# ay-lab/mustache

Measured on AMD Instinct MI355X. Metric: scale-space Mpix/s (sigma-stack+local-max), higher is better.
Workload: dtype f64

## Files before the change

### mustache_amd/csrc/mst_diff.hip

```cpp
#include <cmath>
#include <cstring>
#include <vector>
#include "mst_common.h"
#include "mst_fir.h"

namespace {

constexpr int kThreads = 256;
constexpr int kParts = 256;

__global__ void __launch_bounds__(kThreads)
diff_image_kernel(const double *__restrict__ c1, const double *__restrict__ c2, const uint8_t *__restrict__ nz1,
                  const uint8_t *__restrict__ nz2, int64_t npx, double *__restrict__ cd, uint8_t *__restrict__ nzb,
                  uint32_t *__restrict__ count) {
    const int b = blockIdx.y;
    const int64_t base = (int64_t)b * npx;
    uint32_t local = 0;
    const int64_t stride = (int64_t)gridDim.x * blockDim.x;
    for (int64_t i = (int64_t)blockIdx.x * blockDim.x + threadIdx.x; i < npx; i += stride) {
        const bool t = nz1[base + i] && nz2[base + i];
        cd[base + i] = t ? c1[base + i] - c2[base + i] : 0.0;
        nzb[base + i] = t ? 1 : 0;
        local += t ? 1u : 0u;
    }
#pragma unroll
    for (int o = 32; o > 0; o >>= 1) local += __shfl_xor(local, o, 64);
    if ((threadIdx.x & 63) == 0 && local) atomicAdd(count + b, local);
}

template <int MODE>
__global__ void __launch_bounds__(kThreads)
masked_partial_kernel(const double *__restrict__ a, const double *__restrict__ bimg, const uint8_t *__restrict__ mask,
                      int64_t npx, const double *__restrict__ fit, double *__restrict__ partial) {
    __shared__ double sh[kThreads];
    const int b = blockIdx.y;
    const int64_t base = (int64_t)b * npx;
    const double mean = MODE == 1 ? fit[2 * b] : 0.0;
    double acc = 0.0;
    const int64_t stride = (int64_t)gridDim.x * blockDim.x;
    for (int64_t i = (int64_t)blockIdx.x * blockDim.x + threadIdx.x; i < npx; i += stride) {
        if (mask[base + i]) {
            const double d = a[base + i] - bimg[base + i];
            if (MODE == 0) acc = acc + d;
            else { const double t = d - mean; acc = acc + t * t; }
        }
    }
    sh[threadIdx.x] = acc;
    __syncthreads();
    for (int s = kThreads / 2; s > 0; s >>= 1) {
        if ((int)threadIdx.x < s) sh[threadIdx.x] = sh[threadIdx.x] + sh[threadIdx.x + s];
        __syncthreads();
    }
    if (threadIdx.x == 0) partial[(size_t)b * kParts + blockIdx.x] = sh[0];
}

template <int MODE>
__global__ void __launch_bounds__(kParts)
masked_finish_kernel(const double *__restrict__ partial, const uint32_t *__restrict__ count, double *__restrict__ fit) {
    __shared__ double sh[kParts];
    const int b = blockIdx.x;
    sh[threadIdx.x] = partial[(size_t)b * kParts + threadIdx.x];
    __syncthreads();
    for (int s = kParts / 2; s > 0; s >>= 1) {
        if ((int)threadIdx.x < s) sh[threadIdx.x] = sh[threadIdx.x] + sh[threadIdx.x + s];
        __syncthreads();
    }
    if (threadIdx.x == 0) {
        const double n = (double)count[b];
        if (MODE == 0) fit[2 * b] = sh[0] / n;
        else fit[2 * b + 1] = sqrt(sh[0] / n);
    }
}

__device__ __forceinline__ double ndtr(double a) {
    const double x = a * 0.70710678118654752440;
    const double z = fabs(x);
    if (z < 0.70710678118654752440) return 0.5 + 0.5 * erf(x);
    double y = 0.5 * erfc(z);
    if (x > 0) y = 1.0 - y;
    return y;
}

__global__ void __launch_bounds__(kThreads)
pair_pvalue_kernel(const mst_found *__restrict__ found, uint32_t found_cap, const uint32_t *__restrict__ found_count,
                   const double *__restrict__ g2, const double *__restrict__ g3, const double *__restrict__ fit,
                   int B, int64_t npx, int tested_per_octave, int sample_offset, double *__restrict__ ppair) {
    const int b = blockIdx.y;
    const int fb = b + sample_offset;
    const uint32_t n = found_count[fb];
    if (n > found_cap) return;
    for (uint32_t i = blockIdx.x * blockDim.x + threadIdx.x; i < n; i += gridDim.x * blockDim.x) {
        const mst_found rec = found[(size_t)fb * found_cap + i];
        const int oct = ((int)rec.level - 1) / tested_per_octave;
        const size_t at = ((size_t)oct * B + b) * npx + rec.pixel;
        const double x = g2[at] - g3[at];
        const double loc = fit[2 * ((size_t)oct * B + b)], scale = fit[2 * ((size_t)oct * B + b) + 1];
        double cdf = ndtr((x - loc) / scale);
        if (!isfinite(cdf)) cdf = 1.0;
        if (cdf > 0.5) cdf = 1.0 - cdf;
        ppair[(size_t)fb * found_cap + i] = cdf * 2.0;
    }
}


struct DiffLevels {
    int n_octaves;
    int radius[16][2];
    double taps[16][2][MST_MAX_RADIUS + 1];
};

template <class T, int R>
__device__ __forceinline__ void diff_blur(const double *ct, double *vb, const double (&w)[T::RMAX + 1], int tid,
                                          const double *vsrc, double *vdst, const double *hsrc, double (&g)[T::K]) {
    vpass<T, R>(ct, vb, w, tid, vsrc, vdst, 0);
    __syncthreads();
    hpass<T, R>(hsrc, w, g);
    __syncthreads();
}

template <class T>
__device__ __forceinline__ void diff_blur_dispatch(int r, const double *ct, double *vb, const double (&w)[T::RMAX + 1],
                                                   int tid, const double *vsrc, double *vdst, const double *hsrc,
                                                   double (&g)[T::K]) {
#define MST_CASE(R_)                                                                  \
    case R_:                                                                          \
        if constexpr (R_ <= T::RMAX) diff_blur<T, R_>(ct, vb, w, tid, vsrc, vdst, hsrc, g); \
        break;
    switch (r) {
        MST_CASE(1) MST_CASE(2) MST_CASE(3) MST_CASE(4) MST_CASE(5) MST_CASE(6) MST_CASE(7)
        MST_CASE(8) MST_CASE(9) MST_CASE(10) MST_CASE(11) MST_CASE(12) MST_CASE(13) MST_CASE(14)
        MST_CASE(15) MST_CASE(16) MST_CASE(17) MST_CASE(18) MST_CASE(19) MST_CASE(20) MST_CASE(21)
        MST_CASE(22) MST_CASE(23) MST_CASE(24) MST_CASE(25) MST_CASE(26) MST_CASE(27) MST_CASE(28)
        default: break;
    }
#undef MST_CASE
}


struct BandSource {
    const double *band1, *band2;
    int64_t n;
    int dpx;
    const int64_t *starts;
    const int32_t *tile_list;

    __device__ __forceinline__ int tile_of(int slot) const { return tile_list[slot]; }

    template <class T>
    __device__ __forceinline__ void stage(int b, int Y0, int X0, int CH, double *ct, uint8_t *nzb, int tid) const {
        constexpr int RGR = T::RGR, RGC = T::RGC, RMAX = T::RMAX;
        const int64_t start = starts[b];
        const int dpx = this->dpx;
        const int64_t n = this->n;
        const bool inner = Y0 >= 0 && X0 >= 0 && Y0 + T::CTR <= CH && X0 + T::CTC <= CH;
        auto pixel = [&](double r1, double r2, int off, double &val, bool &both) {
            const bool fill = off <= 4 || off >= dpx + 1;
            both = r1 != 0.0 && r2 != 0.0 && off >= 4;
            val = both ? ((fill ? 2.0 : r1) - (fill ? 2.0 : r2)) : 0.0;
        };
        if (inner) {
            constexpr int ND = T::CTR + T::CTC - 1;
            constexpr int PER = (T::CTR + 63) / 64;
            constexpr int U = 10 / PER > 0 ? 10 / PER : 1;
            for (int q0 = tid >> 6; q0 < ND; q0 += T::NW * U) {
                double a1[U][PER], a2[U][PER];
#pragma unroll
                for (int u = 0; u < U; ++u) {
                    const int q = q0 + u * T::NW;
                    const int dd = q - (T::CTR - 1);
                    const int off = X0 - Y0 + dd;
                    const int i_lo = dd < 0 ? -dd : 0;
                    const int i_hi = T::CTC - dd < T::CTR ? T::CTC - dd : T::CTR;
                    const bool in_band = q < ND && off >= 0 && off <= dpx + 1;
                    const int64_t at = (int64_t)(in_band ? off : 0) * n + start + Y0;
#pragma unroll
                    for (int e = 0; e < PER; ++e) {
                        const int i = i_lo + (tid & 63) + 64 * e;
                        const bool ok = in_band && i < i_hi && start + X0 + i + dd < n;
                        a1[u][e] = ok ? band1[at + i] : 0.0;
                        a2[u][e] = ok ? band2[at + i] : 0.0;
                    }
                }
#pragma unroll
                for (int u = 0; u < U; ++u) {
                    const int q = q0 + u * T::NW;
                    if (q >= ND) break;
                    const int dd = q - (T::CTR - 1);
                    const int off = X0 - Y0 + dd;
                    const int i_lo = dd < 0 ? -dd : 0;
                    const int i_hi = T::CTC - dd < T::CTR ? T::CTC - dd : T::CTR;
#pragma unroll
                    for (int e = 0; e < PER; ++e) {
                        const int i = i_lo + (tid & 63) + 64 * e;
                        if (i >= i_hi) continue;
                        const int j = i + dd;
                        double val;
                        bool both;
                        pixel(a1[u][e], a2[u][e], off, val, both);
                        ct[j * T::CTP + i] = val;
                        const int ri = i - RMAX, rj = j - RMAX;
                        if (ri >= 0 && ri < RGR && rj >= 0 && rj < RGC) nzb[ri * RGC + rj] = both ? 1 : 0;
                    }
                }
            }
        } else {
            for (int idx = tid; idx < T::CTR * T::CTC; idx += T::NT) {
                const int i = idx / T::CTC, j = idx - i * T::CTC;
                const int uy = Y0 + i, ux = X0 + j;
                const int by = reflect_idx(uy, CH), bx = reflect_idx(ux, CH);
                const int off = bx - by;
                double r1 = 0.0, r2 = 0.0;
                if (off >= 0 && off <= dpx + 1 && start + bx < n) {
                    r1 = band1[(int64_t)off * n + start + by];
                    r2 = band2[(int64_t)off * n + start + by];
                }
                double val;
                bool both;
                pixel(r1, r2, off, val, both);
                ct[j * T::CTP + i] = val;
                const int ri = i - RMAX, rj = j - RMAX;
                if (ri >= 0 && ri < RGR && rj >= 0 && rj < RGC) {
                    const bool inside = uy >= 0 && uy < CH && ux >= 0 && ux < CH;
                    nzb[ri * RGC + rj] = (inside && both) ? 1 : 0;
                }
            }
        }
    }
};

struct DenseSource {
    const double *c1, *c2;

    __device__ __forceinline__ int tile_of(int slot) const { return slot; }

    template <class T>
    __device__ __forceinline__ void stage(int b, int Y0, int X0, int CH, double *ct, uint8_t *nzb, int tid) const {
        constexpr int RGR = T::RGR, RGC = T::RGC, RMAX = T::RMAX;
        constexpr int N = T::CTR * T::CTC;
        constexpr int U = 4;
        const double *p1 = c1 + (int64_t)b * CH * CH, *p2 = c2 + (int64_t)b * CH * CH;
        const bool inner = Y0 >= 0 && X0 >= 0 && Y0 + T::CTR <= CH && X0 + T::CTC <= CH;
        for (int i0 = tid; i0 < N; i0 += T::NT * U) {
            double a1[U], a2[U];
#pragma unroll
            for (int u = 0; u < U; ++u) {
                const int idx = i0 + u * T::NT;
                const int i = idx / T::CTC, j = idx - i * T::CTC;
                const int by = inner ? Y0 + i : reflect_idx(Y0 + i, CH), bx = inner ? X0 + j : reflect_idx(X0 + j, CH);
                const int64_t at = (int64_t)by * CH + bx;
                a1[u] = idx < N ? p1[at] : 0.0;
                a2[u] = idx < N ? p2[at] : 0.0;
            }
#pragma unroll
            for (int u = 0; u < U; ++u) {
                const int idx = i0 + u * T::NT;
                if (idx >= N) break;
                const int i = idx / T::CTC, j = idx - i * T::CTC;
                const bool both = a1[u] != 0.0 && a2[u] != 0.0;
                ct[j * T::CTP + i] = both ? a1[u] - a2[u] : 0.0;
                const int ri = i - RMAX, rj = j - RMAX;
                if (ri >= 0 && ri < RGR && rj >= 0 && rj < RGC) {
                    const int uy = Y0 + i, ux = X0 + j;
                    nzb[ri * RGC + rj] = (uy < CH && ux < CH && both) ? 1 : 0;
                }
            }
        }
    }
};

template <class T, class Src>
__global__ void __launch_bounds__(T::NT)
diff_dog_kernel(const Src src, int CH, int B, const DiffLevels *__restrict__ lv, double *__restrict__ dog,
                double *__restrict__ partial, uint32_t *__restrict__ mask_count, int tiles_x, int n_slots) {
    constexpr int K = T::K, RGR = T::RGR, RGC = T::RGC, RMAX = T::RMAX;
    extern __shared__ __align__(16) double lds[];
    double *ct = lds;
    double *vb = ct + T::CT_ELEMS;
    double *red = vb + T::VB_ELEMS;
    const int tid = threadIdx.x, b = blockIdx.y;
    const int per_xcd = gridDim.x >> 3;
    const int slot = (blockIdx.x & 7) * per_xcd + (blockIdx.x >> 3);
    if (slot >= n_slots) return;
    const int tile = src.tile_of(slot);
    const int ty = tile / tiles_x, tx = tile - ty * tiles_x;
    const int y0 = ty * RGR, x0 = tx * RGC;
    const int rr = tid % RGR, cg = tid / RGR;
    const int gy = y0 + rr;

    uint8_t *nzb = reinterpret_cast<uint8_t *>(vb);
    src.template stage<T>(b, y0 - RMAX, x0 - RMAX, CH, ct, nzb, tid);
    __syncthreads();
    uint32_t in_mask = 0, both_mask = 0;
#pragma unroll
    for (int k = 0; k < K; ++k) {
        const int gx = x0 + cg * K + k;
        if (gy < CH && gx < CH) {
            in_mask |= 1u << k;
            if (nzb[rr * RGC + cg * K + k]) both_mask |= 1u << k;
        }
    }
    uint32_t mine = __builtin_popcount(both_mask);
#pragma unroll
    for (int o = 32; o > 0; o >>= 1) mine += __shfl_xor(mine, o, 64);
    if ((tid & 63) == 0 && mine) atomicAdd(mask_count + b, mine);
    __syncthreads();

    constexpr int V_MAINC = T::NT / (T::RGR / K);
    const int v_rgp = tid / V_MAINC, v_col = tid - v_rgp * V_MAINC;
    const double *vsrc = ct + v_col * T::CTP + v_rgp * K;
    double *vdst = vb + (v_rgp * K) * T::VP + v_col;
    const double *hsrc = vb + rr * T::VP + cg * K;
    double *part = partial + (((size_t)b * n_slots + slot) * lv->n_octaves) * 2;
    for (int o = 0; o < lv->n_octaves; ++o) {
        double g2[K], g3[K];
        {
            double taps[RMAX + 1];
#pragma unroll
            for (int j = 0; j <= RMAX; ++j) taps[j] = lv->taps[o][0][j];
            diff_blur_dispatch<T>(lv->radius[o][0], ct, vb, taps, tid, vsrc, vdst, hsrc, g2);
        }
        {
            const DiffLevels *lv3 = lv;
            if constexpr (RMAX > 8) asm volatile("" : "+s"(lv3));
            double taps[RMAX + 1];
#pragma unroll
            for (int j = 0; j <= RMAX; ++j) taps[j] = lv3->taps[o][1][j];
            diff_blur_dispatch<T>(lv3->radius[o][1], ct, vb, taps, tid, vsrc, vdst, hsrc, g3);
        }
        double s1 = 0.0, s2 = 0.0;
        double *out = dog + (((size_t)o * B + b) * CH + gy) * CH + x0 + cg * K;
#pragma unroll
        for (int k = 0; k < K; ++k) {
            const double dk = g2[k] - g3[k];
            if ((in_mask >> k) & 1u) out[k] = dk;
            if ((both_mask >> k) & 1u) {
                s1 = s1 + dk;
                s2 = s2 + dk * dk;
            }
        }
        red[tid] = s1;
        red[T::NT + tid] = s2;
        __syncthreads();
        for (int st = T::NT / 2; st > 0; st >>= 1) {
            if (tid < st) {
                red[tid] = red[tid] + red[tid + st];
                red[T::NT + tid] = red[T::NT + tid] + red[T::NT + tid + st];
            }
            __syncthreads();
        }
        if (tid == 0) {
            part[2 * o] = red[0];
            part[2 * o + 1] = red[T::NT];
        }
        __syncthreads();
    }
}

__global__ void __launch_bounds__(256)
diff_fit_kernel(const double *__restrict__ partial, int ntiles, int n_slots, const int32_t *__restrict__ slot_of_tile,
                int n_oct, int B, const uint32_t *__restrict__ mask_count, double *__restrict__ fit) {
    __shared__ double sa[256], sb[256];
    const int o = blockIdx.x, b = blockIdx.y, tid = threadIdx.x;
    double a = 0.0, q = 0.0;
    for (int i = tid; i < ntiles; i += 256) {
        const int sl = slot_of_tile ? slot_of_tile[i] : i;
        if (sl < 0) continue;
        a = a + partial[(((size_t)b * n_slots + sl) * n_oct + o) * 2];
        q = q + partial[(((size_t)b * n_slots + sl) * n_oct + o) * 2 + 1];
    }
    sa[tid] = a;
    sb[tid] = q;
    __syncthreads();
    for (int st = 128; st > 0; st >>= 1) {
        if (tid < st) {
            sa[tid] = sa[tid] + sa[tid + st];
            sb[tid] = sb[tid] + sb[tid + st];
        }
        __syncthreads();
    }
    if (tid == 0) {
        const double cnt = (double)mask_count[b];
        const double loc = sa[0] / cnt;
        double var = sb[0] / cnt - loc * loc;
        if (var < 0.0) var = 0.0;
        fit[2 * ((size_t)o * B + b)] = loc;
        fit[2 * ((size_t)o * B + b) + 1] = sqrt(var);
    }
}

__global__ void __launch_bounds__(kThreads)
pair_pvalue_dog_kernel(const mst_found *__restrict__ found, uint32_t found_cap, const uint32_t *__restrict__ found_count,
                       const double *__restrict__ dog, const double *__restrict__ fit, int B, int64_t npx,
                       int tested_per_octave, int sample_offset, double *__restrict__ ppair) {
    const int b = blockIdx.y;
    const int fb = b + sample_offset;
    const uint32_t nrec = found_count[fb];
    if (nrec > found_cap) return;
    for (uint32_t i = blockIdx.x * blockDim.x + threadIdx.x; i < nrec; i += gridDim.x * blockDim.x) {
        const mst_found rec = found[(size_t)fb * found_cap + i];
        const int oct = ((int)rec.level - 1) / tested_per_octave;
        const double x = dog[((size_t)oct * B + b) * npx + rec.pixel];
        const double loc = fit[2 * ((size_t)oct * B + b)], scale = fit[2 * ((size_t)oct * B + b) + 1];
        double cdf = ndtr((x - loc) / scale);
        if (!isfinite(cdf)) cdf = 1.0;
        if (cdf > 0.5) cdf = 1.0 - cdf;
        ppair[(size_t)fb * found_cap + i] = cdf * 2.0;
    }
}

using DiffTile8 = Tile<32, 64, 8>;
using DiffTile14 = Tile<32, 64, 14>;
using DiffTile28 = Tile<32, 64, 28, 4, 1, false, true>;

static_assert(DiffTile8::RGR == DiffTile14::RGR && DiffTile14::RGR == DiffTile28::RGR && DiffTile8::RGC == DiffTile14::RGC &&
                  DiffTile14::RGC == DiffTile28::RGC,
              "the three difference tiles share one region shape");

template <class T>
size_t diff_lds_bytes() { return sizeof(double) * (size_t)(T::CT_ELEMS + T::VB_ELEMS + 2 * T::NT); }
template <class T>
int diff_tiles(int CH) { return ((CH + T::RGR - 1) / T::RGR) * ((CH + T::RGC - 1) / T::RGC); }

size_t diff_align(size_t v) { return (v + 255) / 256 * 256; }

int diff_levels(const char *who, const mst_levels *lv, DiffLevels *out, int *max_radius) {
    if (!lv || lv->n_octaves < 1 || lv->n_octaves > 16 || lv->levels_per_octave < 3 ||
        lv->n_octaves * lv->levels_per_octave > MST_MAX_LEVELS)
        return mst::fail(MST_E_ARG, "%s: bad level table (1..16 octaves, >= 3 levels each)", who);
    memset(out, 0, sizeof(*out));
    out->n_octaves = lv->n_octaves;
    int mr = 0;
    for (int o = 0; o < lv->n_octaves; ++o)
        for (int q = 0; q < 2; ++q) {
            const int l = o * lv->levels_per_octave + 1 + q;
            const int r = lv->radius[l];
            if (r < 1 || r > 28) return mst::fail(MST_E_ARG, "%s: blur radius %d outside [1, 28]", who, r);
            out->radius[o][q] = r;
            for (int j = 0; j <= r; ++j) out->taps[o][q][j] = lv->taps[l][j];
            mr = r > mr ? r : mr;
        }
    *max_radius = mr;
    return MST_OK;
}

template <class T>
int diff_tile_list(int CH, int dpx, int32_t *list) {
    const int tx = (CH + T::RGC - 1) / T::RGC, nt = diff_tiles<T>(CH);
    for (int i = 0; i < 2 * nt; ++i) list[i] = -1;
    int m = 0;
    for (int t = 0; t < nt; ++t) {
        const int y0 = (t / tx) * T::RGR, x0 = (t % tx) * T::RGC;
        const int r_hi = y0 + T::RGR - 1 < CH - 1 ? y0 + T::RGR - 1 : CH - 1;
        const int c_hi = x0 + T::RGC - 1 < CH - 1 ? x0 + T::RGC - 1 : CH - 1;
        if (c_hi - y0 >= 4 && x0 - r_hi <= dpx + 1) {
            list[(size_t)nt + t] = m;
            list[(size_t)m++] = t;
        }
    }
    return m;
}

template <class T, class Src>
int diff_dog_launch(const Src &src, const int32_t *slot_of_tile, int CH, int B, const DiffLevels *d_lv, int n_oct, double *dog,
                    double *partial, int m, uint32_t *mask_count, double *fit, hipStream_t s) {
    static unsigned long long lds_allowed = 0;
    MST_HIP(mst::allow_dynamic_lds(reinterpret_cast<const void *>(&diff_dog_kernel<T, Src>), (int)diff_lds_bytes<T>(),
                                   &lds_allowed));
    const int tx = (CH + T::RGC - 1) / T::RGC, nt = diff_tiles<T>(CH);
    if (m > 0) {
        diff_dog_kernel<T, Src><<<dim3((m + 7) / 8 * 8, B), T::NT, diff_lds_bytes<T>(), s>>>(src, CH, B, d_lv, dog, partial,
                                                                                           mask_count, tx, m);
        MST_LAUNCH_CHECK();
    }
    diff_fit_kernel<<<dim3(n_oct, B), 256, 0, s>>>(partial, nt, m, slot_of_tile, n_oct, B, mask_count, fit);
    MST_LAUNCH_CHECK();
    return MST_OK;
}

int diff_which(int max_radius) { return max_radius <= DiffTile8::RMAX ? 0 : (max_radius <= DiffTile14::RMAX ? 1 : 2); }

// ... 235 lines not shown
```

### mustache_amd/csrc/mst_fir.h

```cpp
#pragma once
#include <cstdint>
#include "mst_common.h"

#if defined(MST_PROFILE) && defined(MST_ABLATE_CT)
#define MST_VARIANT(bit_) ((MST_ABLATE_CT) & (bit_))
#elif defined(MST_PROFILE)
#define MST_VARIANT(bit_) (variant & (bit_))
#else
#define MST_VARIANT(bit_) 0
#endif

#ifdef MST_PROFILE
#define MST_TRACE_WGS 64
#define MST_TRACE_STAMPS 8
#define MST_STAMP(tr_, slot_)                                                        \
    if (tr_) {                                                                       \
        const unsigned long long t_ = __builtin_amdgcn_s_memtime();                  \
        if ((threadIdx.x & 63) == 0) (tr_)[slot_] = t_;                              \
    }
#else
#define MST_STAMP(tr_, slot_)
#endif

#ifndef MST_KC8_BELOW
// ... 27 lines not shown
#define MST_INJECT_PASS
#endif

struct DevLevels {
    int n_octaves;
    int levels_per_octave;
    int radius[MST_MAX_LEVELS];
    int first_level[16];
    double taps[MST_MAX_LEVELS][MST_MAX_RADIUS + 1];
};

constexpr int pitch_for(int need) {
    int p = need;
    while (p % 32 != 2 && p % 32 != 30) ++p;
    return p;
}
constexpr int pitch_min(int need) {
    int p = need + (need & 1);
    while ((p / 2) % 2 == 0) p += 2;
    return p;
}

template <int RGR_, int RGC_, int RMAX_, int K_ = 8, int MINW_ = 1, bool FMA_ = false, bool TIGHT_ = false>
struct Tile {
    static constexpr bool FMA = FMA_;
    static constexpr int RGR = RGR_, RGC = RGC_;
    static constexpr int ITR = RGR_ - 2, ITC = RGC_ - 2;
    static constexpr int RMAX = RMAX_;
    static constexpr int K = K_;
    static constexpr int MINW = MINW_;
    static constexpr int NCG = RGC / K;
    static constexpr int NT = RGR * NCG;
    static constexpr int NW = NT / 64;
    static constexpr int CTR = RGR + 2 * RMAX;
    static constexpr int CTC = RGC + 2 * RMAX;
    static constexpr int CTP = TIGHT_ ? pitch_min(CTR) : pitch_for(CTR);
    static constexpr int VP = TIGHT_ ? pitch_min(RGC + 2 * RMAX) : pitch_for(RGC + 2 * RMAX);
    static constexpr int CT_ELEMS = CTC * CTP;
    static constexpr int VB_ELEMS = RGR * VP;
    static constexpr int DE_ELEMS = NCG * 2 * RGR;
    static constexpr int ST_ELEMS = MST_MAX_TESTED * NW * 2;
    static constexpr size_t LDS_BYTES = sizeof(double) * (size_t)(CT_ELEMS + VB_ELEMS + DE_ELEMS + ST_ELEMS);
    static_assert(NT % 64 == 0 && RGR % K == 0 && RGC % K == 0, "whole waves, whole groups");
    static_assert(64 % RGR == 0 || RGR % 64 == 0, "a wave holds whole runs of consecutive rows");
    static_assert(CTP % 2 == 0 && VP % 2 == 0 && CT_ELEMS % 2 == 0 && VB_ELEMS % 2 == 0, "16-byte alignment");
};

__device__ __forceinline__ int reflect_idx(int i, int n) {
    const int p = 2 * n;
    i %= p;
    if (i < 0) i += p;
    return i < n ? i : p - 1 - i;
}

template <int K, int R>
__device__ __forceinline__ void fir_sym(const double (&win)[K + 2 * R], const double (&w)[R + 1], double (&t)[K]) {
#pragma unroll
    for (int k = 0; k < K; ++k) t[k] = win[k + R] * w[0];
#pragma unroll
    for (int j = R; j >= 1; --j) {
        double s[K];
#pragma unroll
        for (int k = 0; k < K; ++k) s[k] = win[k + R - j] + win[k + R + j];
#pragma unroll
        for (int k = 0; k < K; ++k) s[k] = s[k] * w[j];
#pragma unroll
        for (int k = 0; k < K; ++k) t[k] = t[k] + s[k];
    }
}

template <int K, int R>
struct Chunk {
    static constexpr int KC = (K >= 8 && R < MST_KC8_BELOW) ? 8 : (K >= 4 ? 4 : K);
};

#if defined(MST_INJECT)
#define MST_FIR_INJ_TPARAM , int INJ = 0
#define MST_FIR_INJ_PARAM , Inject *inj = nullptr
#else
#define MST_FIR_INJ_TPARAM
#define MST_FIR_INJ_PARAM
#endif
template <int KC, int R, int OFF, bool FMA MST_FIR_INJ_TPARAM>
__device__ __forceinline__ void fir_chunk(const double *__restrict__ p, const double (&w)[R + 1], double (&t)[KC] MST_FIR_INJ_PARAM) {
    constexpr int NP = (KC + 2 * R + OFF + 1) / 2;
    constexpr int QC0 = (R + OFF) >> 1, QC1 = (R + KC - 1 + OFF) >> 1;
    const double2 *p2 = reinterpret_cast<const double2 *>(p);
    double x[2 * NP];
#if defined(MST_PROFILE) && defined(MST_ABL_NOLDS)
#define MST_LD(q_)                                        \
    {                                                     \
        double a_ = w[0], b_ = w[R];                      \
        asm volatile("" : "+v"(a_), "+v"(b_));            \
        x[2 * (q_)] = a_;                                 \
        x[2 * (q_) + 1] = b_;                             \
    }
#else
#define MST_LD(q_)                     \
    {                                  \
        const double2 v_ = p2[q_];     \
        x[2 * (q_)] = v_.x;            \
        x[2 * (q_) + 1] = v_.y;        \
    }
#endif
#pragma unroll
    for (int q = QC0; q <= QC1; ++q) MST_LD(q)
#if defined(MST_INJECT)
    if constexpr (INJ == 3) {
        __builtin_amdgcn_sched_barrier(0);
        inject_work<>(*inj);
        __builtin_amdgcn_sched_barrier(0);
    }
#endif
    int lq_hi = -1, rq_lo = NP;
#pragma unroll
    for (int k = 0; k < KC; ++k) t[k] = x[R + k + OFF] * w[0];
#pragma unroll
    for (int j = R; j >= 1; --j) {
        const int lq1 = (R - j + KC - 1 + OFF) >> 1, rq0 = (R + j + OFF) >> 1;
#pragma unroll
        for (int q = 0; q < NP; ++q) {
            if (q > lq_hi && q <= lq1 && q < QC0) MST_LD(q)
            if (q < rq_lo && q >= rq0 && q > QC1) MST_LD(q)
        }
        lq_hi = lq1 > lq_hi ? lq1 : lq_hi;
        rq_lo = rq0 < rq_lo ? rq0 : rq_lo;
#if defined(MST_INJECT)
        if constexpr (INJ == 4) {
            __builtin_amdgcn_sched_barrier(0);
            inject_work<(MST_INJ_DP + R - 1) / R, (MST_INJ_INT + R - 1) / R>(*inj);
            __builtin_amdgcn_sched_barrier(0);
        }
#endif
#if defined(MST_PROFILE) && defined(MST_ABL_NOMATH)
        if (j & 1) t[j % KC] = t[j % KC] + (x[R - j + OFF] + x[R + KC - 1 + j + OFF]);
#else
        double s[KC];
#pragma unroll
        for (int k = 0; k < KC; ++k) s[k] = x[R + k - j + OFF] + x[R + k + j + OFF];
        if constexpr (FMA) {
#pragma unroll
            for (int k = 0; k < KC; ++k) t[k] = __builtin_fma(s[k], w[j], t[k]);
        } else {
#pragma unroll
            for (int k = 0; k < KC; ++k) s[k] = s[k] * w[j];
#pragma unroll
            for (int k = 0; k < KC; ++k) t[k] = t[k] + s[k];
        }
#endif
    }
#undef MST_LD
}

template <class T, int R>
__device__ __forceinline__ void vpass(const double *__restrict__ ct, double *__restrict__ vb,
                                      const double (&wall)[T::RMAX + 1], int ptid, const double *__restrict__ vsrc,
                                      double *__restrict__ vdst, int variant MST_INJECT_ARG) {
    constexpr int K = T::K, KC = Chunk<T::K, R>::KC;
    constexpr int NC = T::RGC + 2 * R;
    constexpr int NRG = T::RGR / K;
    constexpr int MAINC = T::NT / NRG < NC ? T::NT / NRG : NC;
    constexpr int OFF = (T::RMAX - R) & 1;
    double w[R + 1];
#pragma unroll
    for (int j = 0; j <= R; ++j) w[j] = wall[j];
    static_assert(MAINC == T::NT / NRG, "the main-item mapping below is radius independent");
    if (!MST_VARIANT(16)) {
        const double *p = vsrc + (T::RMAX - R) * T::CTP + (T::RMAX - R - OFF);
        double *q = vdst;
#pragma unroll
        for (int h = 0; h < K / KC; ++h) {
            double t[KC];
#if defined(MST_INJECT) && (MST_INJECT == 3 || MST_INJECT == 4)
            if (h == 0) fir_chunk<KC, R, OFF, T::FMA, MST_INJECT>(p + h * KC, w, t, &inj);
            else
#endif
            fir_chunk<KC, R, OFF, T::FMA>(p + h * KC, w, t);
#pragma unroll
            for (int k = 0; k < KC; ++k) q[(h * KC + k) * T::VP] = t[k];
        }
#if defined(MST_INJECT) && MST_INJECT == 1
        inject_work<>(inj);
#endif
    }
    if constexpr (MAINC < NC) if (!MST_VARIANT(8)) {
        constexpr int PR = 4;
        constexpr int XC = NC - MAINC;
        constexpr int XRG = T::RGR / PR;
        for (int it = ptid; it < XRG * XC; it += T::NT) {
            const int rgp = it / XC;
            const int col = MAINC + (it - rgp * XC);
            const int row0 = rgp * PR;
            const double *p = ct + ((T::RMAX - R) + col) * T::CTP + (row0 + T::RMAX - R - OFF);
            double t[PR];
            fir_chunk<PR, R, OFF, T::FMA>(p, w, t);
            double *q = vb + row0 * T::VP + col;
#pragma unroll
            for (int k = 0; k < PR; ++k) q[k * T::VP] = t[k];
        }
    }
}

template <class T, int R>
__device__ __forceinline__ void hpass(const double *__restrict__ p, const double (&wall)[T::RMAX + 1],
                                      double (&g)[T::K]) {
    constexpr int K = T::K, KC = Chunk<T::K, R>::KC;
    double w[R + 1];
#pragma unroll
    for (int j = 0; j <= R; ++j) w[j] = wall[j];
#pragma unroll
    for (int h = 0; h < K / KC; ++h) {
        double t[KC];
        fir_chunk<KC, R, 0, T::FMA>(p + h * KC, w, t);
#pragma unroll
        for (int k = 0; k < KC; ++k) g[h * KC + k] = t[k];
    }
}

}
```

### mustache_amd/csrc/mst_scale_space.hip

```cpp
#include <algorithm>
#include <climits>
#include <cmath>
#include <cstdlib>
#include <cstring>
#include <vector>
#include "mst_common.h"

#include "mst_fir.h"

namespace {

__device__ __forceinline__ double dmax(double a, double b) { return __builtin_fmax(a, b); }

__device__ __forceinline__ double lane_prev(double x) {
    const int lo = __builtin_amdgcn_update_dpp(0, __double2loint(x), 0x138, 0xf, 0xf, true);
    const int hi = __builtin_amdgcn_update_dpp(0, __double2hiint(x), 0x138, 0xf, 0xf, true);
    return __hiloint2double(hi, lo);
}
__device__ __forceinline__ double lane_next(double x) {
    const int lo = __builtin_amdgcn_update_dpp(0, __double2loint(x), 0x130, 0xf, 0xf, true);
    const int hi = __builtin_amdgcn_update_dpp(0, __double2hiint(x), 0x130, 0xf, 0xf, true);
    return __hiloint2double(hi, lo);
}

template <int CTRL, int ROW_MASK>
__device__ __forceinline__ double dpp_fetch(double x) {
    const int lo = __builtin_amdgcn_mov_dpp(__double2loint(x), CTRL, ROW_MASK, 0xf, true);
    const int hi = __builtin_amdgcn_mov_dpp(__double2hiint(x), CTRL, ROW_MASK, 0xf, true);
    return __hiloint2double(hi, lo);
}
__device__ __forceinline__ void wave_reduce_min_sum(double &mn, double &sm) {
#define MST_STEP(CTRL, MASK)                                           \
    {                                                                  \
        const double a_ = dpp_fetch<CTRL, MASK>(mn);                   \
        const double b_ = dpp_fetch<CTRL, MASK>(sm);                   \
        mn = a_ < mn ? a_ : mn;                                        \
        sm = sm + b_;                                                  \
    }
    MST_STEP(0x111, 0xf)
    MST_STEP(0x112, 0xf)
    MST_STEP(0x114, 0xf)
    MST_STEP(0x118, 0xf)
    MST_STEP(0x142, 0xa)
    MST_STEP(0x143, 0xc)
#undef MST_STEP
}

template <class T, int R>
__device__ __forceinline__ void blur_level(const double *ct, double *vb, const double (&w)[T::RMAX + 1], int tid,
                                           const double *vsrc, double *vdst, const double *hsrc, double (&g)[T::K],
                                           int variant, unsigned long long *tr MST_INJECT_ARG) {
    vpass<T, R>(ct, vb, w, tid, vsrc, vdst, variant MST_INJECT_PASS);
    MST_STAMP(tr, 1)
    __syncthreads();
    MST_STAMP(tr, 2)
    if (MST_VARIANT(32)) {
#pragma unroll
        for (int k = 0; k < T::K; ++k) g[k] = 0.0;
        return;
    }
    hpass<T, R>(hsrc, w, g);
    MST_STAMP(tr, 3)
}

template <class T>
__device__ __forceinline__ void blur_dispatch(int r, const double *ct, double *vb, const double (&wg)[T::RMAX + 1],
                                              int tid, const double *vsrc, double *vdst, const double *hsrc,
                                              double (&g)[T::K], int variant, unsigned long long *tr MST_INJECT_ARG) {
#define MST_CASE(R_)                                                  \
    case R_:                                                          \
        if constexpr (R_ <= T::RMAX) blur_level<T, R_>(ct, vb, wg, tid, vsrc, vdst, hsrc, g, variant, tr MST_INJECT_PASS); \
        break;
    switch (r) {
        MST_CASE(1) MST_CASE(2) MST_CASE(3) MST_CASE(4) MST_CASE(5) MST_CASE(6) MST_CASE(7)
        MST_CASE(8) MST_CASE(9) MST_CASE(10) MST_CASE(11) MST_CASE(12) MST_CASE(13) MST_CASE(14)
        MST_CASE(15) MST_CASE(16) MST_CASE(17) MST_CASE(18) MST_CASE(19) MST_CASE(20) MST_CASE(21)
        MST_CASE(22) MST_CASE(23) MST_CASE(24) MST_CASE(25) MST_CASE(26) MST_CASE(27) MST_CASE(28)
        default: break;
    }
#undef MST_CASE
}

struct BandSrc {
    const double *band;
    int64_t n;
    int dpx;
    const int64_t *starts;
    uint32_t *nz_count;
    const double *band2;
    int split;
};

struct WorkItem {
    int32_t y0, x0, b, delta2;
};

struct KernArgs {
    const double *c;
    const uint8_t *nz;
    BandSrc src;
    int CH;
    const DevLevels *lv;
    mst_found *found;
    uint32_t found_cap;
    uint32_t *found_count;
    double *partial;
    const WorkItem *items;
    int n_items, n_tested, skip_empty, variant;
    unsigned long long *trace;
};

template <class T, bool BAND>
__global__ void __launch_bounds__(T::NT, T::MINW)
scale_space_kernel(const double *__restrict__ c, const uint8_t *__restrict__ nz, BandSrc src, int CH,
                   const DevLevels *__restrict__ lv, mst_found *__restrict__ found, uint32_t found_cap,
                   uint32_t *__restrict__ found_count, double *__restrict__ partial, const WorkItem *__restrict__ items,
                   int n_items, int n_tested, int skip_empty, int variant, unsigned long long *__restrict__ trace) {
    constexpr int K = T::K, RGR = T::RGR, RGC = T::RGC, RMAX = T::RMAX;
    extern __shared__ __align__(16) double lds[];
    double *ct = lds;
    double *vb = ct + T::CT_ELEMS;
    double *de = vb + T::VB_ELEMS;
    double *st = de + T::DE_ELEMS;

    const int tid = threadIdx.x;
    const int per_xcd = gridDim.x >> 3;
    const int slot = (blockIdx.x & 7) * per_xcd + (blockIdx.x >> 3);
    if (slot >= n_items) return;
    const WorkItem item = items[slot];
    const int b = item.b, b2 = item.delta2 != 0 ? item.b + 1 : -1;
    const int y0 = item.y0, x0 = item.x0;

    const int rr = tid % RGR;
    const int cg = tid / RGR;
    const int gy = y0 + rr;
    const bool row_in = gy >= 0 && gy < CH;
    const bool row_own = row_in && rr >= 1 && rr <= T::ITR;
    double *part = partial + (size_t)slot * n_tested * 2;

    uint32_t in_mask = 0, nz_mask = 0;
#pragma unroll
    for (int k = 0; k < K; ++k) {
        const int gx = x0 + cg * K + k;
        if (row_in && gx >= 0 && gx < CH) in_mask |= 1u << k;
    }

    if constexpr (!BAND) {
        const double *cb = c + (size_t)b * CH * CH;
        const uint8_t *nb = nz + (size_t)b * CH * CH;
#pragma unroll
        for (int k = 0; k < K; ++k) {
            const int rc = cg * K + k;
            const int gx = x0 + rc;
            if (row_own && gx >= 0 && gx < CH && rc >= 1 && rc <= T::ITC && nb[(size_t)gy * CH + gx]) nz_mask |= 1u << k;
        }
        const int any_nz = __syncthreads_or(nz_mask != 0);
        if (!any_nz && skip_empty) {
            for (int t = tid; t < n_tested; t += T::NT) {
                part[2 * t] = INFINITY;
                part[2 * t + 1] = 0.0;
            }
            return;
        }
        constexpr int CPL = (T::CTC + 63) / 64;
        int sx[CPL];
#pragma unroll
        for (int q = 0; q < CPL; ++q) sx[q] = reflect_idx(x0 - RMAX + (tid & 63) + 64 * q, CH);
        for (int i = tid >> 6; i < T::CTR; i += T::NW) {
            const double *srow = cb + (size_t)reflect_idx(y0 - RMAX + i, CH) * CH;
#pragma unroll
            for (int q = 0; q < CPL; ++q) {
                const int j = (tid & 63) + 64 * q;
                if (j < T::CTC) ct[j * T::CTP + i] = srow[sx[q]];
            }
        }
        __syncthreads();
    } else {
        const int64_t start = src.starts[b];
        const int64_t n = src.n;
        const int dpx = src.dpx;
        const double *const bandp = b >= src.split ? src.band2 : src.band;
        uint8_t *nzb = reinterpret_cast<uint8_t *>(vb);
        const int Y0 = y0 - RMAX, X0 = x0 - RMAX;
        const bool inner = Y0 >= 0 && X0 >= 0 && Y0 + T::CTR <= CH && X0 + T::CTC <= CH;
        const bool constant = inner && (X0 + T::CTC - 1 - Y0 <= 3 || X0 - (Y0 + T::CTR - 1) >= dpx + 2);
        if (constant) {
            double2 *ct2 = reinterpret_cast<double2 *>(ct);
            for (int i = tid; i < T::CT_ELEMS / 2; i += T::NT) ct2[i] = make_double2(2.0, 2.0);
            uint4 *nz4 = reinterpret_cast<uint4 *>(nzb);
            static_assert((RGR * RGC) % 16 == 0, "nzb is cleared in 16-byte pieces");
            for (int i = tid; i < RGR * RGC / 16; i += T::NT) nz4[i] = make_uint4(0, 0, 0, 0);
        } else if (inner) {
            constexpr int ND = T::CTR + T::CTC - 1;
            constexpr int PER = (T::CTR + 63) / 64;
            constexpr int U2 = (ND + 2 * T::NW - 1) / (2 * T::NW);
            constexpr int U = U2 * PER <= 20 ? U2 : 20 / PER;
            for (int q0 = tid >> 6; q0 < ND; q0 += T::NW * U) {
                double rawv[U][PER];
#pragma unroll
                for (int u = 0; u < U; ++u) {
                    const int q = q0 + u * T::NW;
                    const int dd = q - (T::CTR - 1);
                    const int off = X0 - Y0 + dd;
                    const int i_lo = dd < 0 ? -dd : 0;
                    const int i_hi = T::CTC - dd < T::CTR ? T::CTC - dd : T::CTR;
                    const bool in_band = q < ND && off >= 0 && off <= dpx + 1;
                    const double *brow = bandp + (int64_t)(in_band ? off : 0) * n + start + Y0;
#pragma unroll
                    for (int e = 0; e < PER; ++e) {
                        const int i = i_lo + (tid & 63) + 64 * e;
                        rawv[u][e] = (in_band && i < i_hi && start + X0 + i + dd < n) ? brow[i] : 0.0;
                    }
                }
#pragma unroll
                for (int u = 0; u < U; ++u) {
                    const int q = q0 + u * T::NW;
                    if (q >= ND) break;
                    const int dd = q - (T::CTR - 1);
                    const int off = X0 - Y0 + dd;
                    const int i_lo = dd < 0 ? -dd : 0;
                    const int i_hi = T::CTC - dd < T::CTR ? T::CTC - dd : T::CTR;
                    const bool filled = off <= 4 || off >= dpx + 1;
#pragma unroll
                    for (int e = 0; e < PER; ++e) {
                        const int i = i_lo + (tid & 63) + 64 * e;
                        if (i >= i_hi) continue;
                        const int j = i + dd;
                        const double raw = rawv[u][e];
                        ct[j * T::CTP + i] = filled ? 2.0 : raw;
                        const int ri = i - RMAX, rj = j - RMAX;
                        if (ri >= 0 && ri < RGR && rj >= 0 && rj < RGC)
                            nzb[ri * RGC + rj] = (raw != 0.0 && off >= 4) ? 1 : 0;
                    }
                }
            }
        } else {
            for (int idx = tid; idx < T::CTR * T::CTC; idx += T::NT) {
                const int i = idx / T::CTC, j = idx - i * T::CTC;
                const int uy = Y0 + i, ux = X0 + j;
                const int by = reflect_idx(uy, CH), bx = reflect_idx(ux, CH);
                const int off = bx - by;
                double raw = 0.0;
                if (off >= 0 && off <= dpx + 1 && start + bx < n) raw = bandp[(int64_t)off * n + start + by];
                ct[j * T::CTP + i] = (off <= 4 || off >= dpx + 1) ? 2.0 : raw;
                const int ri = i - RMAX, rj = j - RMAX;
                if (ri >= 0 && ri < RGR && rj >= 0 && rj < RGC) {
                    const bool inside = uy >= 0 && uy < CH && ux >= 0 && ux < CH;
                    nzb[ri * RGC + rj] = (inside && raw != 0.0 && off >= 4) ? 1 : 0;
                }
            }
        }
        __syncthreads();
        uint32_t mine = 0;
#pragma unroll
        for (int k = 0; k < K; ++k) {
            const int rc = cg * K + k;
            if (row_own && ((in_mask >> k) & 1u) && rc >= 1 && rc <= T::ITC && nzb[rr * RGC + rc]) nz_mask |= 1u << k;
        }
        mine = __builtin_popcount(nz_mask);
#pragma unroll
        for (int o = 32; o > 0; o >>= 1) mine += __shfl_xor(mine, o, 64);
        if ((tid & 63) == 0 && mine) {
            atomicAdd(src.nz_count + b, mine);
            if (b2 >= 0) atomicAdd(src.nz_count + b2, mine);
        }
        const int any_nz = __syncthreads_or(nz_mask != 0);
        if (!any_nz && skip_empty) {
            for (int t = tid; t < n_tested; t += T::NT) {
                part[2 * t] = INFINITY;
                part[2 * t + 1] = 0.0;
            }
            return;
        }
    }

    double gprev[K], Dc[K], Mc[K], best[K];
    uint32_t lvl[K];
    uint32_t ep = 0, ec = 0, gp = 0;
#pragma unroll
    for (int k = 0; k < K; ++k) {
        gprev[k] = Dc[k] = Mc[k] = best[k] = 0.0;
        lvl[k] = 0;
    }
    const int wave = tid >> 6, lane = tid & 63;
    const bool wave_has_nz = __any(nz_mask != 0);
    const bool wave_all_in = __all(in_mask == (1u << K) - 1u);
    double *de_mine = de + (cg * 2) * RGR + rr;
    const double *de_left = de + ((cg > 0 ? cg - 1 : 0) * 2 + 1) * RGR + rr;
    const double *de_right = de + ((cg < T::NCG - 1 ? cg + 1 : cg) * 2) * RGR + rr;

    constexpr int V_MAINC = T::NT / (T::RGR / K);
    const int v_rgp = tid / V_MAINC, v_col = tid - v_rgp * V_MAINC;
    const double *vsrc = ct + v_col * T::CTP + v_rgp * K;
    double *vdst = vb + (v_rgp * K) * T::VP + v_col;
    const double *hsrc = vb + rr * T::VP + cg * K;

    const int n_oct = MST_VARIANT(4) ? 0 : lv->n_octaves, lpo = lv->levels_per_octave;
    const int prot = (int)(blockIdx.x >> 3) * 2 + (int)(blockIdx.x >> 11);
    int tested = 0;
#if defined(MST_INJECT)
    Inject inj;
#pragma unroll
    for (int k = 0; k < 8; ++k) {
        inj.q[k] = (double)(tid + k);
        inj.u[k] = (uint32_t)(tid * 7 + k);
    }
#endif
    unsigned long long *tr = nullptr;
#ifdef MST_PROFILE
    if (trace && slot >= 3 * (per_xcd >> 3) && slot < 3 * (per_xcd >> 3) + MST_TRACE_WGS) {
        tr = trace + ((size_t)(slot - 3 * (per_xcd >> 3)) * T::NW + (tid >> 6)) * (MST_MAX_LEVELS + 1) * MST_TRACE_STAMPS;
        MST_STAMP(tr, MST_MAX_LEVELS * MST_TRACE_STAMPS + 1)
        if ((tid & 63) == 0) tr[MST_MAX_LEVELS * MST_TRACE_STAMPS + 2] = (unsigned long long)slot | ((unsigned long long)(nz_mask != 0) << 40);
    }
#endif
    for (int o = 0; o < n_oct; ++o) {
        for (int kl = lv->first_level[o]; kl <= lpo; ++kl) {
            const int l = o * lpo + kl - 1;
            const int r = lv->radius[l];
            MST_STAMP(tr, 0)
            double taps[RMAX + 1];
#pragma unroll
            for (int j = 0; j <= RMAX; ++j) taps[j] = lv->taps[l][j];
            double g[K];
            const int ptid = (tid + 64 * ((l + prot) & 3)) & (T::NT - 1);
            blur_dispatch<T>(r, ct, vb, taps, ptid, vsrc, vdst, hsrc, g, variant, tr MST_INJECT_PASS);
            double d[K];
            if (kl >= 2) {
#pragma unroll
                for (int k = 0; k < K; ++k) d[k] = gprev[k] - g[k];
                if (!wave_all_in) {
#pragma unroll
                    for (int k = 0; k < K; ++k)
                        if (!((in_mask >> k) & 1u)) d[k] = 0.0;
                }
                de_mine[0] = d[0];
                de_mine[RGR] = d[K - 1];
            }
#pragma unroll
            for (int k = 0; k < K; ++k) gprev[k] = g[k];
            MST_STAMP(tr, 4)
            __syncthreads();
            MST_STAMP(tr, 5)
#ifdef MST_PROFILE
            unsigned long long *tr_lvl = tr;
            if (tr) tr += MST_TRACE_STAMPS;
#endif
#if defined(MST_INJECT) && MST_INJECT == 2
            inject_work<>(inj);
#endif
            if (kl < 2) continue;
            if (MST_VARIANT(1) || MST_VARIANT(32)) continue;

            uint32_t en = 0, gn = 0;
            double m[K];
            if (wave_has_nz) {
                const double dl = de_left[0], dr = de_right[0];
                double hm[K];
#pragma unroll
                for (int j = 0; j < K / 2; ++j) {
                    const double pj = dmax(d[2 * j], d[2 * j + 1]);
                    hm[2 * j] = dmax(j == 0 ? dl : d[2 * j - 1], pj);
                    hm[2 * j + 1] = dmax(pj, 2 * j + 2 == K ? dr : d[2 * j + 2]);
                }
#pragma unroll
                for (int k = 0; k < K; ++k) m[k] = dmax(dmax(lane_prev(hm[k]), hm[k]), lane_next(hm[k]));
#pragma unroll
                for (int k = 0; k < K; ++k) {
                    if (d[k] == m[k]) en |= 1u << k;
                    if (d[k] > Mc[k]) gn |= 1u << k;
                }
            } else {
#pragma unroll
                for (int k = 0; k < K; ++k) m[k] = 0.0;
            }
            if (kl >= 4) {
                double lmin = INFINITY, lsum = 0.0;
                const uint32_t code = (uint32_t)tested + 1u;
                if (wave_has_nz) {
                    const uint32_t flags = nz_mask & ec & (ep | en) & gp;
#pragma unroll
                    for (int k = 0; k < K; ++k) {
                        const bool bit = (flags & (1u << k)) != 0;
                        const bool upd = bool(int(Dc[k] > dmax(best[k], m[k])) & int(bit));
                        best[k] = upd ? Dc[k] : best[k];
                        lvl[k] = upd ? code : lvl[k];
                        const bool tz = (nz_mask & (1u << k)) != 0;
                        const double a = fabs(Dc[k]);
                        lmin = __builtin_fmin(lmin, tz ? a : INFINITY);
                        lsum = lsum + (tz ? a : 0.0);
                    }
                }
                if (wave_has_nz && !MST_VARIANT(2)) wave_reduce_min_sum(lmin, lsum);
                if (lane == 63) {
                    st[(tested * T::NW + wave) * 2] = lmin;
                    st[(tested * T::NW + wave) * 2 + 1] = lsum;
                }
                ++tested;
            }
            ep = ec;
            ec = en;
            gp = gn;
#pragma unroll
            for (int k = 0; k < K; ++k) {
                Mc[k] = m[k];
                Dc[k] = d[k];
            }
#ifdef MST_PROFILE
            MST_STAMP(tr_lvl, 6)
#endif
        }
    }

    int e_b = b, e_b2 = b2, e_x0 = x0, e_delta2 = item.delta2, e_CH = CH;
    if constexpr (T::RMAX > 14) {
        typedef const KernArgs __attribute__((address_space(4))) *KernArgsPtr;
        KernArgsPtr ka = (KernArgsPtr)__builtin_amdgcn_kernarg_segment_ptr();
        found = ka->found;
        found_cap = ka->found_cap;
        found_count = ka->found_count;
        n_tested = ka->n_tested;
        part = ka->partial + (size_t)slot * n_tested * 2;
        const WorkItem again = ka->items[slot];
        e_b = again.b;
        e_b2 = again.delta2 != 0 ? again.b + 1 : -1;
        e_x0 = again.x0;
        e_delta2 = again.delta2;
        e_CH = ka->CH;
    }
#if defined(MST_INJECT)
    {
        double qs = 0.0;
        uint32_t us = 0;
#pragma unroll
        for (int k = 0; k < 8; ++k) {
            qs += inj.q[k];
            us ^= inj.u[k];
        }
        if (qs == -1.0 && us == 0x12345u) part[0] = qs;
    }
#endif
    uint32_t my_total = 0;
    uint32_t before[K];
    uint32_t kbase[K];
#pragma unroll
    for (int k = 0; k < K; ++k) {
        const unsigned long long bal = __ballot(lvl[k] != 0);
        before[k] = __builtin_popcountll(bal & ((1ull << lane) - 1ull));
        kbase[k] = my_total;
        my_total += (uint32_t)__builtin_popcountll(bal);
    }
    uint32_t *cnt_lds = reinterpret_cast<uint32_t *>(de);
    __syncthreads();
    if (lane == 0) cnt_lds[wave] = my_total;
    __syncthreads();
    if (tid == 0) {
        uint32_t tot = 0;
        for (int w = 0; w < T::NW; ++w) {
            const uint32_t n = cnt_lds[w];
            cnt_lds[w] = tot;
            tot += n;
        }
        cnt_lds[T::NW] = tot ? atomicAdd(found_count + e_b, tot) : 0u;
        cnt_lds[T::NW + 1] = (tot && e_b2 >= 0) ? atomicAdd(found_count + e_b2, tot) : 0u;
    }
    __syncthreads();
    const uint32_t wave_base = cnt_lds[T::NW] + cnt_lds[wave];
    const uint32_t wave_base2 = cnt_lds[T::NW + 1] + cnt_lds[wave];
#pragma unroll
    for (int k = 0; k < K; ++k) {
        if (lvl[k]) {
            const uint32_t off = kbase[k] + before[k];
            mst_found rec;
            rec.pixel = (uint32_t)gy * (uint32_t)e_CH + (uint32_t)(e_x0 + cg * K + k);
            rec.level = lvl[k];
            rec.value = best[k];
            if (wave_base + off < found_cap) found[(size_t)e_b * found_cap + wave_base + off] = rec;
            if (e_b2 >= 0 && wave_base2 + off < found_cap) {
                rec.pixel = (uint32_t)(gy + e_delta2) * (uint32_t)e_CH + (uint32_t)(e_x0 + cg * K + k + e_delta2);
// ... 644 lines not shown
```

Baseline: 18030.

## Remap vertical-pass edge pieces to bank-conflict-free lane layout with precomputed addresses

Replaces the strided loop over extra (halo) column pieces in the vertical FIR pass with a fixed lane-to-piece mapping. At most one piece goes to each lane, chosen per wave, and a constexpr check proves the LDS loads and stores are free of bank conflicts. Per-thread source and destination addresses are precomputed once in a VAddr struct, and the rotating piece owner becomes a wave-uniform scalar via readfirstlane. The aim is to remove LDS bank conflicts and the loop and division overhead in the halo work, at the cost of a more rigid mapping that only holds for 8-row-group tile shapes.

```diff
diff --git a/mustache_amd/csrc/mst_diff.hip b/mustache_amd/csrc/mst_diff.hip
--- a/mustache_amd/csrc/mst_diff.hip
+++ b/mustache_amd/csrc/mst_diff.hip
@@ -110,21 +110,20 @@
 };
 
 template <class T, int R>
-__device__ __forceinline__ void diff_blur(const double *ct, double *vb, const double (&w)[T::RMAX + 1], int tid,
-                                          const double *vsrc, double *vdst, const double *hsrc, double (&g)[T::K]) {
-    vpass<T, R>(ct, vb, w, tid, vsrc, vdst, 0);
+__device__ __forceinline__ void diff_blur(const double *ct, const double (&w)[T::RMAX + 1], int pwave, const VAddr &va,
+                                          const double *hsrc, double (&g)[T::K]) {
+    vpass<T, R>(ct, w, pwave, va, 0);
     __syncthreads();
     hpass<T, R>(hsrc, w, g);
     __syncthreads();
 }
 
 template <class T>
-__device__ __forceinline__ void diff_blur_dispatch(int r, const double *ct, double *vb, const double (&w)[T::RMAX + 1],
-                                                   int tid, const double *vsrc, double *vdst, const double *hsrc,
-                                                   double (&g)[T::K]) {
+__device__ __forceinline__ void diff_blur_dispatch(int r, const double *ct, const double (&w)[T::RMAX + 1], int pwave,
+                                                   const VAddr &va, const double *hsrc, double (&g)[T::K]) {
 #define MST_CASE(R_)                                                                  \
     case R_:                                                                          \
-        if constexpr (R_ <= T::RMAX) diff_blur<T, R_>(ct, vb, w, tid, vsrc, vdst, hsrc, g); \
+        if constexpr (R_ <= T::RMAX) diff_blur<T, R_>(ct, w, pwave, va, hsrc, g); \
         break;
     switch (r) {
         MST_CASE(1) MST_CASE(2) MST_CASE(3) MST_CASE(4) MST_CASE(5) MST_CASE(6) MST_CASE(7)
@@ -305,10 +304,8 @@
     if ((tid & 63) == 0 && mine) atomicAdd(mask_count + b, mine);
     __syncthreads();
 
-    constexpr int V_MAINC = T::NT / (T::RGR / K);
-    const int v_rgp = tid / V_MAINC, v_col = tid - v_rgp * V_MAINC;
-    const double *vsrc = ct + v_col * T::CTP + v_rgp * K;
-    double *vdst = vb + (v_rgp * K) * T::VP + v_col;
+    const VAddr va = vpass_addr<T>(ct, vb, tid);
+    const int pwave = __builtin_amdgcn_readfirstlane(tid >> 6);
     const double *hsrc = vb + rr * T::VP + cg * K;
     double *part = partial + (((size_t)b * n_slots + slot) * lv->n_octaves) * 2;
     for (int o = 0; o < lv->n_octaves; ++o) {
@@ -317,7 +314,7 @@
             double taps[RMAX + 1];
 #pragma unroll
             for (int j = 0; j <= RMAX; ++j) taps[j] = lv->taps[o][0][j];
-            diff_blur_dispatch<T>(lv->radius[o][0], ct, vb, taps, tid, vsrc, vdst, hsrc, g2);
+            diff_blur_dispatch<T>(lv->radius[o][0], ct, taps, pwave, va, hsrc, g2);
         }
         {
             const DiffLevels *lv3 = lv;
@@ -325,7 +322,7 @@
             double taps[RMAX + 1];
 #pragma unroll
             for (int j = 0; j <= RMAX; ++j) taps[j] = lv3->taps[o][1][j];
-            diff_blur_dispatch<T>(lv3->radius[o][1], ct, vb, taps, tid, vsrc, vdst, hsrc, g3);
+            diff_blur_dispatch<T>(lv3->radius[o][1], ct, taps, pwave, va, hsrc, g3);
         }
         double s1 = 0.0, s2 = 0.0;
         double *out = dog + (((size_t)o * B + b) * CH + gy) * CH + x0 + cg * K;
diff --git a/mustache_amd/csrc/mst_fir.h b/mustache_amd/csrc/mst_fir.h
--- a/mustache_amd/csrc/mst_fir.h
+++ b/mustache_amd/csrc/mst_fir.h
@@ -203,10 +203,51 @@
 #undef MST_LD
 }
 
+constexpr int piece_col(int lane) { return lane & 7; }
+constexpr int piece_rgp(int lane) {
+    return 2 * (lane >> 5) + 4 * ((lane >> 4) & 1) + (((((lane & 31) + 4) >> 3) ^ (lane >> 4)) & 1);
+}
+constexpr int b128_group(int lane) {
+    const int m = lane & 31;
+    return 2 * (lane >> 5) + ((m >= 4 && m < 12) || (m >= 16 && m < 20) || m >= 28 ? 1 : 0);
+}
+constexpr bool vpass_map_ok(int ctp, int vp) {
+    unsigned long long seen = 0;
+    for (int l = 0; l < 64; ++l) {
+        const int id = piece_rgp(l) * 8 + piece_col(l);
+        if (piece_rgp(l) < 0 || piece_rgp(l) > 7 || ((seen >> id) & 1)) return false;
+        seen |= 1ull << id;
+    }
+    for (int a = 0; a < 64; ++a)
+        for (int b = a + 1; b < 64; ++b) {
+            const int ra = piece_col(a) * ctp + 4 * piece_rgp(a), rb = piece_col(b) * ctp + 4 * piece_rgp(b);
+            if (b128_group(a) == b128_group(b) && (ra / 2) % 16 == (rb / 2) % 16) return false;
+            const int wa = 4 * piece_rgp(a) * vp + piece_col(a), wb = 4 * piece_rgp(b) * vp + piece_col(b);
+            if (a / 16 == b / 16 && wa % 16 == wb % 16) return false;
+        }
+    return true;
+}
+
+struct VAddr {
+    const double *vsrc, *psrc;
+    double *vdst, *pdst;
+};
+template <class T>
+__device__ __forceinline__ VAddr vpass_addr(const double *ct, double *vb, int tid) {
+    constexpr int MAINC = T::NT / (T::RGR / T::K);
+    const int v_rgp = tid / MAINC, v_col = tid - v_rgp * MAINC;
+    const int pc = MAINC + piece_col(tid & 63), prow = 4 * piece_rgp(tid & 63);
+    VAddr a;
+    a.vsrc = ct + v_col * T::CTP + v_rgp * T::K;
+    a.vdst = vb + (v_rgp * T::K) * T::VP + v_col;
+    a.psrc = ct + pc * T::CTP + prow;
+    a.pdst = vb + prow * T::VP + pc;
+    return a;
+}
+
 template <class T, int R>
-__device__ __forceinline__ void vpass(const double *__restrict__ ct, double *__restrict__ vb,
-                                      const double (&wall)[T::RMAX + 1], int ptid, const double *__restrict__ vsrc,
-                                      double *__restrict__ vdst, int variant MST_INJECT_ARG) {
+__device__ __forceinline__ void vpass(const double *__restrict__ ct, const double (&wall)[T::RMAX + 1], int pwave,
+                                      const VAddr &va, int variant MST_INJECT_ARG) {
     constexpr int K = T::K, KC = Chunk<T::K, R>::KC;
     constexpr int NC = T::RGC + 2 * R;
     constexpr int NRG = T::RGR / K;
@@ -217,8 +258,8 @@
     for (int j = 0; j <= R; ++j) w[j] = wall[j];
     static_assert(MAINC == T::NT / NRG, "the main-item mapping below is radius independent");
     if (!MST_VARIANT(16)) {
-        const double *p = vsrc + (T::RMAX - R) * T::CTP + (T::RMAX - R - OFF);
-        double *q = vdst;
+        const double *p = va.vsrc + (T::RMAX - R) * T::CTP + (T::RMAX - R - OFF);
+        double *q = va.vdst;
 #pragma unroll
         for (int h = 0; h < K / KC; ++h) {
             double t[KC];
@@ -237,17 +278,18 @@
     if constexpr (MAINC < NC) if (!MST_VARIANT(8)) {
         constexpr int PR = 4;
         constexpr int XC = NC - MAINC;
-        constexpr int XRG = T::RGR / PR;
-        for (int it = ptid; it < XRG * XC; it += T::NT) {
-            const int rgp = it / XC;
-            const int col = MAINC + (it - rgp * XC);
-            const int row0 = rgp * PR;
-            const double *p = ct + ((T::RMAX - R) + col) * T::CTP + (row0 + T::RMAX - R - OFF);
-            double t[PR];
-            fir_chunk<PR, R, OFF, T::FMA>(p, w, t);
-            double *q = vb + row0 * T::VP + col;
-#pragma unroll
-            for (int k = 0; k < PR; ++k) q[k * T::VP] = t[k];
+        static_assert(T::RGR == 8 * PR && XC <= 8 * T::NW, "piece_col / piece_rgp: 8 row groups, at most one piece per lane");
+        static_assert(vpass_map_ok(T::CTP, T::VP), "the pieces' window loads and stores are free of LDS bank conflicts");
+        if (8 * pwave < XC) {
+            const double *p0 = va.psrc + pwave * (8 * T::CTP);
+            if (p0 < ct + (MAINC + XC) * T::CTP) {
+                const double *p = p0 + (T::RMAX - R) * T::CTP + (T::RMAX - R - OFF);
+                double t[PR];
+                fir_chunk<PR, R, OFF, T::FMA>(p, w, t);
+                double *q = va.pdst + pwave * 8;
+#pragma unroll
+                for (int k = 0; k < PR; ++k) q[k * T::VP] = t[k];
+            }
         }
     }
 }
diff --git a/mustache_amd/csrc/mst_scale_space.hip b/mustache_amd/csrc/mst_scale_space.hip
--- a/mustache_amd/csrc/mst_scale_space.hip
+++ b/mustache_amd/csrc/mst_scale_space.hip
@@ -47,10 +47,10 @@
 }
 
 template <class T, int R>
-__device__ __forceinline__ void blur_level(const double *ct, double *vb, const double (&w)[T::RMAX + 1], int tid,
-                                           const double *vsrc, double *vdst, const double *hsrc, double (&g)[T::K],
-                                           int variant, unsigned long long *tr MST_INJECT_ARG) {
-    vpass<T, R>(ct, vb, w, tid, vsrc, vdst, variant MST_INJECT_PASS);
+__device__ __forceinline__ void blur_level(const double *ct, const double (&w)[T::RMAX + 1], int pwave, const VAddr &va,
+                                           const double *hsrc, double (&g)[T::K], int variant,
+                                           unsigned long long *tr MST_INJECT_ARG) {
+    vpass<T, R>(ct, w, pwave, va, variant MST_INJECT_PASS);
     MST_STAMP(tr, 1)
     __syncthreads();
     MST_STAMP(tr, 2)
@@ -64,12 +64,12 @@
 }
 
 template <class T>
-__device__ __forceinline__ void blur_dispatch(int r, const double *ct, double *vb, const double (&wg)[T::RMAX + 1],
-                                              int tid, const double *vsrc, double *vdst, const double *hsrc,
-                                              double (&g)[T::K], int variant, unsigned long long *tr MST_INJECT_ARG) {
+__device__ __forceinline__ void blur_dispatch(int r, const double *ct, const double (&wg)[T::RMAX + 1], int pwave,
+                                              const VAddr &va, const double *hsrc, double (&g)[T::K], int variant,
+                                              unsigned long long *tr MST_INJECT_ARG) {
 #define MST_CASE(R_)                                                  \
     case R_:                                                          \
-        if constexpr (R_ <= T::RMAX) blur_level<T, R_>(ct, vb, wg, tid, vsrc, vdst, hsrc, g, variant, tr MST_INJECT_PASS); \
+        if constexpr (R_ <= T::RMAX) blur_level<T, R_>(ct, wg, pwave, va, hsrc, g, variant, tr MST_INJECT_PASS); \
         break;
     switch (r) {
         MST_CASE(1) MST_CASE(2) MST_CASE(3) MST_CASE(4) MST_CASE(5) MST_CASE(6) MST_CASE(7)
@@ -289,10 +289,7 @@
     const double *de_left = de + ((cg > 0 ? cg - 1 : 0) * 2 + 1) * RGR + rr;
     const double *de_right = de + ((cg < T::NCG - 1 ? cg + 1 : cg) * 2) * RGR + rr;
 
-    constexpr int V_MAINC = T::NT / (T::RGR / K);
-    const int v_rgp = tid / V_MAINC, v_col = tid - v_rgp * V_MAINC;
-    const double *vsrc = ct + v_col * T::CTP + v_rgp * K;
-    double *vdst = vb + (v_rgp * K) * T::VP + v_col;
+    const VAddr va = vpass_addr<T>(ct, vb, tid);
     const double *hsrc = vb + rr * T::VP + cg * K;
 
     const int n_oct = MST_VARIANT(4) ? 0 : lv->n_octaves, lpo = lv->levels_per_octave;
@@ -323,8 +320,8 @@
 #pragma unroll
             for (int j = 0; j <= RMAX; ++j) taps[j] = lv->taps[l][j];
             double g[K];
-            const int ptid = (tid + 64 * ((l + prot) & 3)) & (T::NT - 1);
-            blur_dispatch<T>(r, ct, vb, taps, ptid, vsrc, vdst, hsrc, g, variant, tr MST_INJECT_PASS);
+            const int pwave = __builtin_amdgcn_readfirstlane((wave + ((l + prot) & 3)) & (T::NW - 1));
+            blur_dispatch<T>(r, ct, taps, pwave, va, hsrc, g, variant, tr MST_INJECT_PASS);
             double d[K];
             if (kl >= 2) {
 #pragma unroll
```

Result: no change. 17980 (-0.3%).
